# StefanHeng/Symbolic-Music-Generation

Measured on AMD Instinct MI355X. Metric: train tokens/sec (TransfoXL seq2048 bf16), whole job, higher is better.
Workload: dtype bf16; 1 GPU; TransfoXL 12L/768d H12 dh64 F3072 T=2048 M=2048 V=1190 cutoffs=[] (SURVEY C3, mode R: fresh zero mems); per_gpu_batch=64, global_batch=64, seq_len=2048, mem_len=2048, parallelism=dp1

## Files before the change

symbolic_music_generation_amd/csrc/gemm.hip:

```cpp
#include <stdlib.h>
#include <type_traits>
#include "common.h"
#include "musicxl_internal.h"

namespace {

constexpr int BM = 128, BK = 64;
constexpr int TILE_BYTES = BM * BK * 2;

struct GemmP {
    const bf16_t* A; const bf16_t* B; void* C;
    int M, N, K, lda, ldb, ldc;
    int ksplit;
    const float* bias;
    const bf16_t* aux;
    int ldaux;
    float alpha;
    int flags;
    unsigned long long seed; unsigned site; unsigned thresh; float drop_scale;
    int tiles_m, tiles_n;
    int bdiv;
    long long sA1, sA2, sB1, sB2, sC1, sC2;
    float* colsum;
    const bf16_t* hd_o; int hd_ldo, hd_T; float* hd_delta;
};
constexpr int GEMM_COLSUM_BIT = 0x80;
constexpr int GEMM_HEADDOT_BIT = 0x400;

typedef __attribute__((address_space(3))) bf16x4 lds_bf16x4;
typedef __attribute__((ext_vector_type(8))) __bf16 mfma_bf16x8;

__device__ __forceinline__ int swzT(int k) { return (k & 3) | (((k >> 3) & 1) << 2); }

template <bool T, int R_>
__device__ __forceinline__ void g2r(const bf16_t* __restrict__ X, int ld, int R, int kend, int r0, int k0, u32x4 (&v)[R_ / 32]) {
    const int t = threadIdx.x;
    constexpr int RC = R_ / 8;
#pragma unroll
    for (int i = 0; i < R_ / 32; i++) {
        const int c = t + i * 256;
        u32x4 z = {0u, 0u, 0u, 0u};
        if (!T) {
            const int row = c >> 3, kc = c & 7;
            const int gr = r0 + row, gk = k0 + kc * 8;
            const bool ok = (gr < R) && (gk < kend);
            v[i] = ok ? *reinterpret_cast<const u32x4*>(X + (size_t)gr * ld + gk) : z;
        } else {
            const int kr = c / RC, rc = c % RC;
            const int gk = k0 + kr, gr = r0 + rc * 8;
            const bool ok = (gk < kend) && (gr < R);
            v[i] = ok ? *reinterpret_cast<const u32x4*>(X + (size_t)gk * ld + gr) : z;
        }
    }
}

template <bool T, int R_>
__device__ __forceinline__ void r2s(char* base, const u32x4 (&v)[R_ / 32]) {
    const int t = threadIdx.x;
    constexpr int RC = R_ / 8;
#pragma unroll
    for (int i = 0; i < R_ / 32; i++) {
        const int c = t + i * 256;
        int off;
        if (!T) {
            const int row = c >> 3, kc = c & 7;
            off = row * 128 + ((kc ^ ((row >> 1) & 7)) << 4);
        } else {
            const int kr = c / RC, rc = c % RC;
            off = kr * (R_ * 2) + (((rc >> 1) ^ (swzT(kr) & (R_ / 16 - 1))) << 5) + ((rc & 1) << 4);
        }
        *reinterpret_cast<u32x4*>(base + off) = v[i];
    }
}

template <bool T, int R_>
__device__ __forceinline__ bf16x8 ldfrag(const char* base, int rb, int ks) {
    const int l = threadIdx.x & 63;
    const int g = l >> 4, li = l & 15;
    if (!T) {
        const int row = rb + li;
        const int chunk = ks * 4 + g;
        return *reinterpret_cast<const bf16x8*>(base + row * 128 + ((chunk ^ ((row >> 1) & 7)) << 4));
    } else {
        const int q = li >> 2, pp = li & 3;
        const int krow = ks * 32 + 8 * g + q;
        const int col = rb + 4 * pp;
        const int off = krow * (R_ * 2) + (((col >> 4) ^ (swzT(krow) & (R_ / 16 - 1))) << 5) + ((col & 15) << 1);
        const lds_bf16x4* p0 = (const lds_bf16x4*)(base + off);
        const lds_bf16x4* p1 = (const lds_bf16x4*)(base + off + 4 * (R_ * 2));
        bf16x4 lo = __builtin_amdgcn_ds_read_tr16_b64_v4i16((lds_bf16x4*)p0);
        bf16x4 hi = __builtin_amdgcn_ds_read_tr16_b64_v4i16((lds_bf16x4*)p1);
        bf16x8 r = {lo[0], lo[1], lo[2], lo[3], hi[0], hi[1], hi[2], hi[3]};
        return r;
    }
}

__device__ __forceinline__ void epilogue_vals(const GemmP& p, const int flags, const int m, const int n, const f32x4 a4_, float (&v)[4],
                                              const uint32_t* auxq = nullptr, const float* biasq = nullptr) {
#pragma unroll
            for (int r = 0; r < 4; r++) v[r] = a4_[r] * p.alpha;
            const bool full = (n + 3 < p.N);
            if ((flags & MXL_GEMM_BIAS) && biasq) {
#pragma unroll
                for (int r = 0; r < 4; r++) v[r] += biasq[r];
            } else if (flags & MXL_GEMM_BIAS) {
                if (full) {
                    const float b0 = p.bias[n], b1 = p.bias[n + 1], b2 = p.bias[n + 2], b3 = p.bias[n + 3];
                    v[0] += b0; v[1] += b1; v[2] += b2; v[3] += b3;
                } else {
#pragma unroll
                    for (int r = 0; r < 4; r++) if (n + r < p.N) v[r] += p.bias[n + r];
                }
            }
            if (flags & MXL_GEMM_RELU) {
#pragma unroll
                for (int r = 0; r < 4; r++) v[r] = fmaxf(v[r], 0.f);
            }
            if (flags & MXL_GEMM_DROPOUT) {
                const uint32_t i0 = (uint32_t)m * (uint32_t)p.N + (uint32_t)n;
                const uint32_t mix = mxl_hash32((uint32_t)p.seed ^ (p.site * 0x9E3779B9U)) + (uint32_t)(p.seed >> 32);
                const uint32_t h0 = i0 * 0x9E3779B1U;
                if (flags & MXL_GEMM_RELU) {
                    const uint32_t t16 = p.thresh >> 16;
#pragma unroll
                    for (int k = 0; k < 2; k++) {
                        const uint32_t h = mxl_hash32((h0 + (uint32_t)(2 * k) * 0x9E3779B1U) ^ mix);
                        v[2 * k] = ((h & 0xffffu) >= t16) ? v[2 * k] * p.drop_scale : 0.f;
                        v[2 * k + 1] = ((h >> 16) >= t16) ? v[2 * k + 1] * p.drop_scale : 0.f;
                    }
                } else
#pragma unroll
                for (int r = 0; r < 4; r++)
                    v[r] = (mxl_hash32((h0 + (uint32_t)r * 0x9E3779B1U) ^ mix) >= p.thresh) ? v[r] * p.drop_scale : 0.f;
            }
            if ((flags & MXL_GEMM_RELU_BWD) && auxq) {
                v[0] = bf2f((bf16_t)(auxq[0] & 0xffffu)) > 0.f ? v[0] : 0.f;
                v[1] = bf2f((bf16_t)(auxq[0] >> 16)) > 0.f ? v[1] : 0.f;
                v[2] = bf2f((bf16_t)(auxq[1] & 0xffffu)) > 0.f ? v[2] : 0.f;
                v[3] = bf2f((bf16_t)(auxq[1] >> 16)) > 0.f ? v[3] : 0.f;
            } else if (flags & MXL_GEMM_RELU_BWD) {
                if (full && ((p.ldaux & 3) == 0)) {
                    const bf16x4 a4 = *reinterpret_cast<const bf16x4*>(p.aux + (size_t)m * p.ldaux + n);
#pragma unroll
                    for (int r = 0; r < 4; r++) v[r] = bf2f((bf16_t)a4[r]) > 0.f ? v[r] : 0.f;
                } else {
#pragma unroll
                    for (int r = 0; r < 4; r++)
                        if (n + r < p.N) {
                            const float a = bf2f(p.aux[(size_t)m * p.ldaux + n + r]);
                            v[r] = a > 0.f ? v[r] : 0.f;
                        }
                }
            }
            if ((flags & MXL_GEMM_ADD_AUX) && auxq) {
                v[0] += bf2f((bf16_t)(auxq[0] & 0xffffu)); v[1] += bf2f((bf16_t)(auxq[0] >> 16));
                v[2] += bf2f((bf16_t)(auxq[1] & 0xffffu)); v[3] += bf2f((bf16_t)(auxq[1] >> 16));
            } else if (flags & MXL_GEMM_ADD_AUX) {
                if (full && ((p.ldaux & 3) == 0)) {
                    const bf16x4 a4 = *reinterpret_cast<const bf16x4*>(p.aux + (size_t)m * p.ldaux + n);
#pragma unroll
                    for (int r = 0; r < 4; r++) v[r] += bf2f((bf16_t)a4[r]);
                } else {
#pragma unroll
                    for (int r = 0; r < 4; r++)
                        if (n + r < p.N) v[r] += bf2f(p.aux[(size_t)m * p.ldaux + n + r]);
                }
            }
}
__device__ __forceinline__ void epilogue_store(const GemmP& p, const int flags, const int m, const int n, const float (&v)[4]) {
            const bool full = (n + 3 < p.N);
            if (flags & MXL_GEMM_OUT_F32_ATOMIC) {
                float* c = reinterpret_cast<float*>(p.C) + (size_t)m * p.ldc + n;
#pragma unroll
                for (int r = 0; r < 4; r++) if (n + r < p.N) atomicAdd(c + r, v[r]);
            } else if (flags & MXL_GEMM_OUT_F32) {
                float* c = reinterpret_cast<float*>(p.C) + (size_t)m * p.ldc + n;
                if (full && ((p.ldc & 3) == 0)) {
                    *reinterpret_cast<f32x4*>(c) = f32x4{v[0], v[1], v[2], v[3]};
                } else {
#pragma unroll
                    for (int r = 0; r < 4; r++) if (n + r < p.N) c[r] = v[r];
                }
            } else {
                bf16_t* c = reinterpret_cast<bf16_t*>(p.C) + (size_t)m * p.ldc + n;
                if (full && ((p.ldc & 3) == 0)) {
                    u32x2 o = {pack2bf(v[0], v[1]), pack2bf(v[2], v[3])};
                    if (flags & (1 << 30)) __builtin_nontemporal_store(o, reinterpret_cast<u32x2*>(c));
                    else *reinterpret_cast<u32x2*>(c) = o;
                } else {
#pragma unroll
                    for (int r = 0; r < 4; r++) if (n + r < p.N) c[r] = f2bf(v[r]);
                }
            }
}
__device__ __forceinline__ void epilogue_quad(const GemmP& p, const int flags, const int m, const int n, const f32x4 a4_) {
    float v[4];
    epilogue_vals(p, flags, m, n, a4_, v);
    epilogue_store(p, flags, m, n, v);
}
__device__ __forceinline__ u32x4 pair_aux_load(const GemmP& p, const int m, const int n, const int l) {
    const int acol = ((l >> 4) & 1) ? n + 16 - 4 : n;
    return *reinterpret_cast<const u32x4*>(p.aux + (size_t)m * p.ldaux + acol);
}
__device__ __forceinline__ void epilogue_pair_bf16(const GemmP& p, const int flags, const int m, const int n, const int l,
                                                   const f32x4 q0, const f32x4 q1, float* cs0 = nullptr, float* cs1 = nullptr,
                                                   const bool have_ax = false, const u32x4 axv = u32x4{0u, 0u, 0u, 0u},
                                                   const float* bq0 = nullptr, const float* bq1 = nullptr,
                                                   const int mask_mode = 0, uint32_t* mbits = nullptr, const int mshift = 0) {
    float v0[4], v1[4];
    if (mask_mode == 2) {
        const uint32_t b = *mbits >> mshift;
#pragma unroll
        for (int r = 0; r < 4; r++) {
            v0[r] = (b >> r) & 1u ? q0[r] * p.alpha : 0.f;
            v1[r] = (b >> (4 + r)) & 1u ? q1[r] * p.alpha : 0.f;
        }
    } else
    if ((flags & (MXL_GEMM_RELU_BWD | MXL_GEMM_ADD_AUX)) && (p.ldaux & 7) == 0 && (reinterpret_cast<uintptr_t>(p.aux) & 15) == 0) {
        const u32x4 ax = have_ax ? axv : pair_aux_load(p, m, n, l);
        const auto s0 = __builtin_amdgcn_permlane16_swap(ax[0], ax[2], false, false);
        const auto s1 = __builtin_amdgcn_permlane16_swap(ax[1], ax[3], false, false);
        const uint32_t aq0[2] = {s0[0], s1[0]}, aq1[2] = {s0[1], s1[1]};
        epilogue_vals(p, flags, m, n, q0, v0, aq0, bq0);
        epilogue_vals(p, flags, m, n + 16, q1, v1, aq1, bq1);
    } else {
        epilogue_vals(p, flags, m, n, q0, v0, nullptr, bq0);
        epilogue_vals(p, flags, m, n + 16, q1, v1, nullptr, bq1);
    }
    if (mask_mode == 1) {
        uint32_t b = 0;
#pragma unroll
        for (int r = 0; r < 4; r++) b |= (v0[r] > 0.f ? 1u << r : 0u) | (v1[r] > 0.f ? 16u << r : 0u);
        *mbits |= b << mshift;
    }
    if (cs0) {
#pragma unroll
        for (int r = 0; r < 4; r++) { cs0[r] += v0[r]; cs1[r] += v1[r]; }
    }
    unsigned a0 = pack2bf(v0[0], v0[1]), a1 = pack2bf(v0[2], v0[3]), b0 = pack2bf(v1[0], v1[1]), b1 = pack2bf(v1[2], v1[3]);
    const auto r0 = __builtin_amdgcn_permlane16_swap(a0, b0, false, false);
    const auto r1 = __builtin_amdgcn_permlane16_swap(a1, b1, false, false);
    const int col = ((l >> 4) & 1) ? n + 16 - 4 : n;
    bf16_t* c = reinterpret_cast<bf16_t*>(p.C) + (size_t)m * p.ldc + col;
    *reinterpret_cast<u32x4*>(c) = u32x4{r0[0], r1[0], r0[1], r1[1]};
}

__device__ __forceinline__ void epilogue_rowpair_bf16(const GemmP& p, const int flags, const int m, const int n, const int l,
                                                      const f32x4 q0, const f32x4 q1) {
    float v0[4], v1[4];
    epilogue_vals(p, flags, m, n, q0, v0);
    epilogue_vals(p, flags, m + 16, n, q1, v1);
    unsigned a0 = pack2bf(v0[0], v0[1]), a1 = pack2bf(v0[2], v0[3]), b0 = pack2bf(v1[0], v1[1]), b1 = pack2bf(v1[2], v1[3]);
    const auto r0 = __builtin_amdgcn_permlane16_swap(a0, b0, false, false);
    const auto r1 = __builtin_amdgcn_permlane16_swap(a1, b1, false, false);
    const bool odd = (l >> 4) & 1;
    bf16_t* c = reinterpret_cast<bf16_t*>(p.C) + (size_t)(odd ? m + 16 : m) * p.ldc + (odd ? n - 4 : n);
    *reinterpret_cast<u32x4*>(c) = u32x4{r0[0], r1[0], r0[1], r1[1]};
}

template <bool AT, bool BT, int BN_, bool SWAP = false>
__global__ __launch_bounds__(256, 2) void gemm_bf16_kernel(GemmP p) {
    constexpr int BN = BN_;
    constexpr int NF = BN / 32;
    constexpr int B_BYTES = BN * BK * 2;
    constexpr int STAGE = TILE_BYTES + B_BYTES;
    extern __shared__ __attribute__((aligned(16))) char smem[];
    const int nwg = p.tiles_m * p.tiles_n;
    int bid = blockIdx.x;
    {
        const int q = nwg >> 3, r = nwg & 7, xcd = bid & 7, idx = bid >> 3;
        bid = (xcd < r ? xcd * (q + 1) : r * (q + 1) + (xcd - r) * q) + idx;
    }
    if (gridDim.y > 1) {
        const long long b1 = blockIdx.y / p.bdiv, b2 = blockIdx.y % p.bdiv;
        p.A += b1 * p.sA1 + b2 * p.sA2;
        p.B += b1 * p.sB1 + b2 * p.sB2;
        const long long co = b1 * p.sC1 + b2 * p.sC2;
        if (p.flags & (MXL_GEMM_OUT_F32 | MXL_GEMM_OUT_F32_ATOMIC)) p.C = reinterpret_cast<float*>(p.C) + co;
        else p.C = reinterpret_cast<bf16_t*>(p.C) + co;
    }
    const int tm = bid / p.tiles_n, tn = bid % p.tiles_n;
    const int m0 = tm * BM, n0 = tn * BN;
    const int kbeg = blockIdx.z * p.ksplit;
    const int kend = min(p.K, kbeg + p.ksplit);
    const int nk = (kend - kbeg + BK - 1) / BK;

    const int wid = threadIdx.x >> 6, l = threadIdx.x & 63;
    const int wr = wid >> 1, wc = wid & 1;

    f32x4 acc[4][NF];
#pragma unroll
    for (int i = 0; i < 4; i++)
#pragma unroll
        for (int j = 0; j < NF; j++) acc[i][j] = f32x4{0.f, 0.f, 0.f, 0.f};

    u32x4 ra[4], rb[BN / 32];
    g2r<AT, 128>(p.A, p.lda, p.M, kend, m0, kbeg, ra);
    g2r<BT, BN>(p.B, p.ldb, p.N, kend, n0, kbeg, rb);
    r2s<AT, 128>(smem, ra);
    r2s<BT, BN>(smem + TILE_BYTES, rb);
    __syncthreads();

    int cur = 0;
    for (int kt = 0; kt < nk; kt++) {
        const bool more = (kt + 1 < nk);
        if (more) {
            g2r<AT, 128>(p.A, p.lda, p.M, kend, m0, kbeg + (kt + 1) * BK, ra);
            g2r<BT, BN>(p.B, p.ldb, p.N, kend, n0, kbeg + (kt + 1) * BK, rb);
        }
        const char* sa = smem + cur * STAGE;
        const char* sb = sa + TILE_BYTES;
#pragma unroll
        for (int ks = 0; ks < 2; ks++) {
            bf16x8 fa[4], fb[NF];
#pragma unroll
            for (int i = 0; i < 4; i++) fa[i] = ldfrag<AT, 128>(sa, wr * 64 + i * 16, ks);
#pragma unroll
            for (int j = 0; j < NF; j++) fb[j] = ldfrag<BT, BN>(sb, wc * (BN / 2) + j * 16, ks);
#pragma unroll
            for (int i = 0; i < 4; i++)
#pragma unroll
                for (int j = 0; j < NF; j++)
                    acc[i][j] = SWAP ? __builtin_amdgcn_mfma_f32_16x16x32_bf16(__builtin_bit_cast(mfma_bf16x8, fa[i]),
                                                                               __builtin_bit_cast(mfma_bf16x8, fb[j]), acc[i][j], 0, 0, 0)
                                     : __builtin_amdgcn_mfma_f32_16x16x32_bf16(__builtin_bit_cast(mfma_bf16x8, fb[j]),
                                                                               __builtin_bit_cast(mfma_bf16x8, fa[i]), acc[i][j], 0, 0, 0);
        }
        if (more) {
            char* da = smem + (cur ^ 1) * STAGE;
            r2s<AT, 128>(da, ra);
            r2s<BT, BN>(da + TILE_BYTES, rb);
        }
        __syncthreads();
        cur ^= 1;
    }

    if (SWAP) {
        float* C = reinterpret_cast<float*>(p.C);
#pragma unroll
        for (int i = 0; i < 4; i++)
#pragma unroll
            for (int j = 0; j < NF; j++) {
                const int n = n0 + wc * (BN / 2) + j * 16 + (l & 15);
#pragma unroll
                for (int r = 0; r < 4; r++) {
                    const int m = m0 + wr * 64 + i * 16 + (l >> 4) * 4 + r;
                    if (m < p.M && n < p.N) atomicAdd(C + (size_t)m * p.ldc + n, acc[i][j][r] * p.alpha);
                }
            }
        return;
    }
    const int flags = p.flags;
    const int mrow_l = l & 15, nq = (l >> 4) * 4;
#pragma unroll
    for (int i = 0; i < 4; i++) {
        const int m = m0 + wr * 64 + i * 16 + mrow_l;
        if (m >= p.M) continue;
#pragma unroll
        for (int j = 0; j < NF; j++) {
            const int n = n0 + wc * (BN / 2) + j * 16 + nq;
            if (n >= p.N) continue;
            epilogue_quad(p, flags, m, n, acc[i][j]);
        }
    }
}

constexpr int G2_OP_BYTES = 256 * 32 * 2;
constexpr int G2_STAGE = 2 * G2_OP_BYTES;
constexpr int G2_SMEM = 4 * G2_STAGE;

__device__ __forceinline__ int g2_swz(int rb) { return ((((rb ^ (rb >> 1)) & 1) << 1) | (rb >> 1)) & 3; }

typedef __attribute__((address_space(1))) const void* g2_gptr;
typedef __attribute__((address_space(3))) void* g2_lptr;

#ifndef NT_ABL
#define NT_ABL 0
#endif
template <int NFN, int EPI = -1>
__global__ __launch_bounds__(512) void gemm_nt256_kernel(GemmP p) {
    constexpr int BN = 64 * NFN;
    constexpr bool PF_ACROSS = !(EPI >= 0 && (EPI & (MXL_GEMM_DROPOUT | 0x100)));
    constexpr int WN = 4, WM = 2;
    constexpr int FM = 16 / WM, FN = BN / 16 / WN;
    extern __shared__ __attribute__((aligned(1024))) char smem[];
    const int nwg = p.tiles_m * p.tiles_n;
    const int G = gridDim.x;
    int bid = blockIdx.x;
    {
        const int q = G >> 3, r = G & 7, xcd = bid & 7, idx = bid >> 3;
        bid = (xcd < r ? xcd * (q + 1) : r * (q + 1) + (xcd - r) * q) + idx;
    }
    const int nk = p.K >> 5;
    const int my_tiles = (nwg - bid + G - 1) / G;
    const int S = my_tiles * nk;

    const int wid = __builtin_amdgcn_readfirstlane(threadIdx.x >> 6), l = threadIdx.x & 63;
    const int wr = wid / WN, wc = wid % WN;

    const __amdgpu_buffer_rsrc_t a_rsrc = __builtin_amdgcn_make_buffer_rsrc((void*)p.A, 0, -1, 0x00020000);
    const __amdgpu_buffer_rsrc_t b_rsrc = __builtin_amdgcn_make_buffer_rsrc((void*)p.B, 0, -1, 0x00020000);
    unsigned ga[2], gb[2];
    int gi = 0, i_t = 0, i_tile = bid;
    auto set_ptrs = [&](int tile) {
        const int tm = tile / p.tiles_n, tn = tile % p.tiles_n;
        const int kc = ((l & 3) ^ g2_swz(l >> 4)) * 8;
#pragma unroll
        for (int i = 0; i < 2; i++) {
            const int row = (8 * i + wid) * 16 + (l >> 2);
            ga[i] = (unsigned)min(tm * 256 + row, p.M - 1) * (unsigned)p.lda + kc;
            gb[i] = (unsigned)min(tn * BN + row, p.N - 1) * (unsigned)p.ldb + kc;
        }
    };
    set_ptrs(i_tile);
    auto issue_next = [&]() {
        char* st = smem + (gi & 3) * G2_STAGE;
        const int k0 = i_t << 5;
#pragma unroll
        for (int i = 0; i < 2; i++) {
            __builtin_amdgcn_raw_ptr_buffer_load_lds(a_rsrc, (g2_lptr)(st + (8 * i + wid) * 1024), 16, (int)((ga[i] + k0) * 2u), 0, 0, 0);
            if (NFN == 4 || i == 0 || wid < 4)
                __builtin_amdgcn_raw_ptr_buffer_load_lds(b_rsrc, (g2_lptr)(st + G2_OP_BYTES + (8 * i + wid) * 1024), 16,
                                                         (int)((gb[i] + k0) * 2u), 0, 0, 0);
        }
        gi++;
        if (++i_t == nk) {
            i_t = 0;
            i_tile += G;
            if (i_tile < nwg) set_ptrs(i_tile);
        }
    };
    const int fsw = ((l >> 4) ^ g2_swz((l >> 2) & 3)) << 4;
    const int a_off = (wr * (FM * 16) + (l & 15)) * 64 + fsw;
    const int b_off = G2_OP_BYTES + (wc * (FN * 16) + (l & 15)) * 64 + fsw;
    auto frags = [&](int g, bf16x8 (&fa)[FM], bf16x8 (&fb)[FN]) {
        const char* st = smem + (g & 3) * G2_STAGE;
#pragma unroll
        for (int j = 0; j < FN; j++) fb[j] = *reinterpret_cast<const bf16x8*>(st + b_off + j * 1024);
#pragma unroll
        for (int i = 0; i < FM; i++) fa[i] = *reinterpret_cast<const bf16x8*>(st + a_off + i * 1024);
    };

    f32x4 acc[FM][FN];
    issue_next();
    if (S > 1) issue_next();
    if (S > 2) issue_next();
    const bool three = (NFN == 3) && wid >= 4;
    if (S > 2) { if (three) asm volatile("s_waitcnt vmcnt(3)" ::: "memory"); else asm volatile("s_waitcnt vmcnt(4)" ::: "memory"); }
    else asm volatile("s_waitcnt vmcnt(0)" ::: "memory");
    __builtin_amdgcn_s_barrier();

    bf16x8 fa0[FM], fb0[FN], fa1[FM], fb1[FN];
    frags(0, fa0, fb0);
    __builtin_amdgcn_s_waitcnt(0xc07f);

    int g = 0;
    auto step = [&](bool first_of_later_tile, bool last_of_tile, bf16x8 (&fa)[FM], bf16x8 (&fb)[FN], bf16x8 (&na)[FM],
                    bf16x8 (&nb)[FN]) {
        const bool issued = gi < S;
        const bool late = wid >= 4;
        if (!late) {
            if (issued && !(NT_ABL & 1)) issue_next();
            if (g + 1 < S && !(last_of_tile && !PF_ACROSS) && !(NT_ABL & 2)) frags(g + 1, na, nb);
        }
        __builtin_amdgcn_s_setprio(1);
#pragma unroll
        for (int i = 0; i < FM; i++)
#pragma unroll
            for (int j = 0; j < FN; j++)
                acc[i][j] = __builtin_amdgcn_mfma_f32_16x16x32_bf16(__builtin_bit_cast(mfma_bf16x8, fb[j]),
                                                                    __builtin_bit_cast(mfma_bf16x8, fa[i]), acc[i][j], 0, 0, 0);
        __builtin_amdgcn_s_setprio(0);
        if (late) {
            __builtin_amdgcn_sched_barrier(0);
            if (g + 1 < S && !(last_of_tile && !PF_ACROSS) && !(NT_ABL & 2)) frags(g + 1, na, nb);
            if (issued && !(NT_ABL & 1)) issue_next();
        }
        if (last_of_tile || !issued) asm volatile("s_waitcnt vmcnt(0)" ::: "memory");
        else if (!first_of_later_tile) {
            if (three) asm volatile("s_waitcnt vmcnt(3)" ::: "memory"); else asm volatile("s_waitcnt vmcnt(4)" ::: "memory");
        }
        if (!(NT_ABL & 4)) __builtin_amdgcn_s_barrier();
        if (NT_ABL & 1) gi++;
        g++;
    };

    constexpr bool BIAS_INIT = EPI >= 0 && (EPI & MXL_GEMM_BIAS);
    const int flags = EPI >= 0 ? (BIAS_INIT ? EPI & ~MXL_GEMM_BIAS : EPI) : p.flags;
    if (EPI == 0 || BIAS_INIT) p.alpha = 1.f;
#pragma unroll 1
    for (int tile = bid; tile < nwg; tile += G) {
        if (BIAS_INIT) {
            const int nb0 = (tile % p.tiles_n) * BN + wc * (FN * 16) + (l >> 4) * 4;
#pragma unroll
            for (int j = 0; j < FN; j++) {
                f32x4 b4;
                const int n = nb0 + j * 16;
                if (n + 3 < p.N) b4 = *reinterpret_cast<const f32x4*>(p.bias + n);
                else
#pragma unroll
                    for (int r = 0; r < 4; r++) b4[r] = n + r < p.N ? p.bias[n + r] : 0.f;
#pragma unroll
                for (int i = 0; i < FM; i++) acc[i][j] = b4;
            }
        } else {
#pragma unroll
            for (int i = 0; i < FM; i++)
#pragma unroll
                for (int j = 0; j < FN; j++) acc[i][j] = f32x4{0.f, 0.f, 0.f, 0.f};
        }
#pragma unroll 1
        for (int t = 0; t < nk; t += 2) {
            step(t == 0 && tile != bid, false, fa0, fb0, fa1, fb1);
            step(false, t + 2 >= nk, fa1, fb1, fa0, fb0);
        }
        const int m0 = (tile / p.tiles_n) * 256, n0 = (tile % p.tiles_n) * BN;
        const bool pairs = !(flags & MXL_GEMM_OUT_F32) && n0 + BN <= p.N && m0 + 256 <= p.M && (p.ldc & 7) == 0 &&
                           (reinterpret_cast<uintptr_t>(p.C) & 15) == 0;
        if (pairs) {
            constexpr bool CS = EPI >= 0 && (EPI & GEMM_COLSUM_BIT) && !(FN & 1);
            float cs[CS ? FN : 1][4];
            if (CS) {
#pragma unroll
                for (int j = 0; j < FN; j++)
#pragma unroll
                    for (int r = 0; r < 4; r++) cs[j][r] = 0.f;
            }
            constexpr bool HA = false && EPI >= 0 && (EPI & (MXL_GEMM_RELU_BWD | MXL_GEMM_ADD_AUX)) && !(FN & 1);
            constexpr int MM = (EPI >= 0 && (EPI & 0x100)) ? 1 : (EPI >= 0 && (EPI & 0x200)) ? 2 : 0;
            uint32_t mb[4] = {0u, 0u, 0u, 0u};
            if (MM == 2) {
                const u32x4 t4 = *(reinterpret_cast<const u32x4*>(p.aux) + ((size_t)tile * 8 + wid) * 64 + l);
                mb[0] = t4[0]; mb[1] = t4[1]; mb[2] = t4[2]; mb[3] = t4[3];
            }
            const bool aux_ok = HA && (p.ldaux & 7) == 0 && (reinterpret_cast<uintptr_t>(p.aux) & 15) == 0;
            u32x4 axn[HA ? FN / 2 : 1];
#pragma unroll
            for (int i = 0; i < FM; i++) {
                const int m = m0 + wr * (FM * 16) + i * 16 + (l & 15);
                u32x4 axc[HA ? FN / 2 : 1];
                if (aux_ok) {
#pragma unroll
                    for (int j = 0; j + 1 < FN; j += 2) {
                        axc[j / 2] = i >= 2 ? axn[j / 2] : pair_aux_load(p, m, n0 + wc * (FN * 16) + j * 16 + (l >> 4) * 4, l);
                        if (i >= 1 && i + 1 < FM) axn[j / 2] = pair_aux_load(p, m + 16, n0 + wc * (FN * 16) + j * 16 + (l >> 4) * 4, l);
                    }
                }
#pragma unroll
                for (int j = 0; j + 1 < FN; j += 2)
                    epilogue_pair_bf16(p, flags & ~(GEMM_COLSUM_BIT | 0x300), m, n0 + wc * (FN * 16) + j * 16 + (l >> 4) * 4, l, acc[i][j], acc[i][j + 1],
                                       CS ? cs[CS ? j : 0] : nullptr, CS ? cs[CS ? j + 1 : 0] : nullptr,
                                       aux_ok, axc[HA ? j / 2 : 0], nullptr, nullptr,
                                       MM, &mb[(i * FN / 2 + j / 2) / 4], 8 * ((i * FN / 2 + j / 2) & 3));
                if ((FN & 1) && !(i & 1))
                    epilogue_rowpair_bf16(p, flags, m, n0 + wc * (FN * 16) + (FN - 1) * 16 + (l >> 4) * 4, l, acc[i][FN - 1],
                                          acc[(i + 1) % FM][FN - 1]);
                if (MM == 1) __builtin_amdgcn_sched_barrier(0);
            }
            if (MM == 1)
                *(reinterpret_cast<u32x4*>(const_cast<bf16_t*>(p.aux)) + ((size_t)tile * 8 + wid) * 64 + l) = u32x4{mb[0], mb[1], mb[2], mb[3]};
            if (CS) {
#pragma unroll
                for (int j = 0; j < FN; j++)
#pragma unroll
                    for (int r = 0; r < 4; r++) {
                        float v = cs[j][r];
                        v += __builtin_bit_cast(float, __builtin_amdgcn_update_dpp(0, __builtin_bit_cast(int, v), 0x128, 0xf, 0xf, false));
                        v += __builtin_bit_cast(float, __builtin_amdgcn_update_dpp(0, __builtin_bit_cast(int, v), 0x124, 0xf, 0xf, false));
                        v += __builtin_bit_cast(float, __builtin_amdgcn_update_dpp(0, __builtin_bit_cast(int, v), 0x122, 0xf, 0xf, false));
                        v += __builtin_bit_cast(float, __builtin_amdgcn_update_dpp(0, __builtin_bit_cast(int, v), 0x121, 0xf, 0xf, false));
                        cs[j][r] = v;
                    }
                if ((l & 15) == 0) {
#pragma unroll
                    for (int j = 0; j < FN; j++)
#pragma unroll
                        for (int r = 0; r < 4; r++) atomicAdd(p.colsum + n0 + wc * (FN * 16) + j * 16 + (l >> 4) * 4 + r, cs[j][r]);
                }
            }
        } else {
#pragma unroll
            for (int i = 0; i < FM; i++) {
                const int m = m0 + wr * (FM * 16) + i * 16 + (l & 15);
                if (m >= p.M) continue;
#pragma unroll
                for (int j = 0; j < FN; j++) {
                    const int n = n0 + wc * (FN * 16) + j * 16 + (l >> 4) * 4;
                    if (n >= p.N) continue;
                    epilogue_quad(p, flags, m, n, acc[i][j]);
                }
            }
        }
        if (!PF_ACROSS && g < S) {
            frags(g, fa0, fb0);
            __builtin_amdgcn_s_waitcnt(0xc07f);
        }
    }
}


#define W4S_(x) #x
#define W4S(x) W4S_(x)
#define W4_AREG(lo, hi) "{a[" W4S(lo) ":" W4S(hi) "]}"
#define W4_MFMA(i, j, lo, hi)                                                                                                     \
    do {                                                                                                                          \
        if (FIRST) asm volatile("v_mfma_f32_16x16x32_bf16 %0, %1, %2, 0" : "=" W4_AREG(lo, hi)(acc[i][j]) : "v"(fb[j]), "v"(fa[i])); \
        else asm volatile("v_mfma_f32_16x16x32_bf16 %0, %1, %2, %0" : "+" W4_AREG(lo, hi)(acc[i][j]) : "v"(fb[j]), "v"(fa[i]));     \
    } while (0)
#define W4_ACC_READ(i, j, r0, r1, r2, r3, lo, hi, q_)                                                                             \
    do {                                                                                                                          \
        float x0_, x1_, x2_, x3_;                                                                                                 \
        asm volatile("v_accvgpr_read_b32 %0, a" W4S(r0) "\n\tv_accvgpr_read_b32 %1, a" W4S(r1) "\n\tv_accvgpr_read_b32 %2, a" W4S(r2)  \
                     "\n\tv_accvgpr_read_b32 %3, a" W4S(r3)                                                                       \
                     : "=&v"(x0_), "=&v"(x1_), "=&v"(x2_), "=&v"(x3_) : W4_AREG(lo, hi)(acc[i][j]));                               \
        q_ = f32x4{x0_, x1_, x2_, x3_};                                                                                           \
    } while (0)
#include "gemm_w4_gen.inc"
template <int OFF>
__device__ __forceinline__ void w4_read(bf16x8& dst, uint32_t addr) {
    asm volatile("ds_read_b128 %0, %1 offset:%2" : "=v"(dst) : "v"(addr), "n"(OFF) : "memory");
}
template <int N>
__device__ __forceinline__ void w4_rd(bf16x8 (&na)[8], bf16x8 (&nb)[8], uint32_t aa, uint32_t bb) {
#if defined(W4_ABL) && (W4_ABL & 2)
    return;
#endif
    if (N < 8) w4_read<(N & 7) * 1024>(nb[N & 7], bb);
    else w4_read<(N & 7) * 1024>(na[N & 7], aa);
}
template <int EPI = -1>
__global__ __launch_bounds__(256, 1) void gemm_nt256w4_kernel(GemmP p) {
    constexpr int BN = 256, FM = 8, FN = 8;
    extern __shared__ __attribute__((aligned(1024))) char smem[];
    const int nwg = p.tiles_m * p.tiles_n;
    const int G = gridDim.x;
    int bid = blockIdx.x;
    {
        const int q = G >> 3, r = G & 7, xcd = bid & 7, idx = bid >> 3;
        bid = (xcd < r ? xcd * (q + 1) : r * (q + 1) + (xcd - r) * q) + idx;
    }
    const int nk = p.K >> 5;
    const int my_tiles = (nwg - bid + G - 1) / G;
    const int S = my_tiles * nk;
    const int wid = __builtin_amdgcn_readfirstlane(threadIdx.x >> 6), l = threadIdx.x & 63;
    const int wr = wid >> 1, wc = wid & 1;

    const __amdgpu_buffer_rsrc_t a_rsrc = __builtin_amdgcn_make_buffer_rsrc((void*)p.A, 0, -1, 0x00020000);
    const __amdgpu_buffer_rsrc_t b_rsrc = __builtin_amdgcn_make_buffer_rsrc((void*)p.B, 0, -1, 0x00020000);
    unsigned ga0, ga1, ga2, ga3, gb0, gb1, gb2, gb3;
    int gi = 0, i_t = 0, i_tile = bid;
    const int kc2 = ((l & 3) ^ g2_swz(l >> 4)) * 16;
#define W4_SET_PTRS(tile_)                                                                                                        \
    do {                                                                                                                          \
        const int tm_ = (tile_) / p.tiles_n, tn_ = (tile_) % p.tiles_n;                                                           \
        const int r0_ = wid * 16 + (l >> 2);                                                                                      \
        ga0 = (unsigned)min(tm_ * 256 + r0_, p.M - 1) * (unsigned)(p.lda * 2) + kc2;       \
        ga1 = (unsigned)min(tm_ * 256 + r0_ + 64, p.M - 1) * (unsigned)(p.lda * 2) + kc2;                                          \
        ga2 = (unsigned)min(tm_ * 256 + r0_ + 128, p.M - 1) * (unsigned)(p.lda * 2) + kc2;                                         \
        ga3 = (unsigned)min(tm_ * 256 + r0_ + 192, p.M - 1) * (unsigned)(p.lda * 2) + kc2;                                         \
        gb0 = (unsigned)min(tn_ * BN + r0_, p.N - 1) * (unsigned)(p.ldb * 2) + kc2;                                                \
// ... 318 lines not shown
}
static bool nt256_use192(int M, int N) {
    const int n_cu = gemm_n_cu();
    const int tm = (M + 255) / 256;
    const int t256 = tm * ((N + 255) / 256), t192 = tm * ((N + 191) / 192);
    const long long c256 = (long long)((t256 + n_cu - 1) / n_cu) * 256, c192 = (long long)((t192 + n_cu - 1) / n_cu) * 192;
    return c192 < c256;
}

extern "C" size_t mxl_gemm_relu_mask_bytes(int M, int N) {
    if (M <= 0 || N <= 0 || (M % 256) != 0 || (N % 256) != 0 || nt256_use192(M, N)) return 0;
    return (size_t)(M / 256) * (size_t)(N / 256) * 8 * 64 * 16;
}

static int gemm_launch(const void* A, const void* B, void* C, int M, int N, int K, int lda, int ldb, int ldc,
                       int transA, int transB, int flags, float alpha, const float* bias,
                       const void* aux, int ldaux, int ksplits,
                       float drop_p, unsigned long long seed, unsigned site, void* stream,
                       int batch, int bdiv, long long sA1, long long sA2, long long sB1, long long sB2,
                       long long sC1, long long sC2, float* colsum = nullptr, bool* colsum_fused = nullptr,
                       const void* hd_o = nullptr, int hd_ldo = 0, int hd_T = 0, float* hd_delta = nullptr, bool* hd_fused = nullptr) {
    MXL_CHECK_ARG(A && B && C && M > 0 && N > 0 && K > 0);
    g_last_nt_kernel = 0;
    MXL_CHECK_ARG((lda % 8) == 0 && (ldb % 8) == 0);
    MXL_CHECK_ARG(((uintptr_t)A % 16) == 0 && ((uintptr_t)B % 16) == 0);
    if (!transA || !transB) MXL_CHECK_ARG((K % 8) == 0);
    MXL_CHECK_ARG(transA ? lda >= ((M + 7) & ~7) : lda >= K);
    MXL_CHECK_ARG(transB ? ldb >= ((N + 7) & ~7) : ldb >= K);
    MXL_CHECK_ARG(ldc >= N);
    if (flags & MXL_GEMM_BIAS) MXL_CHECK_ARG(bias != nullptr);
    if (flags & (MXL_GEMM_SAVE_RELU_MASK | MXL_GEMM_RELU_BWD_BITS)) {
        MXL_CHECK_ARG(aux != nullptr && ((uintptr_t)aux & 15) == 0 && !(flags & (MXL_GEMM_RELU_BWD | MXL_GEMM_ADD_AUX)));
        MXL_CHECK_ARG(!((flags & MXL_GEMM_SAVE_RELU_MASK) && (flags & MXL_GEMM_RELU_BWD_BITS)));
        if (mxl_gemm_relu_mask_bytes(M, N) == 0 || transA || transB || batch != 1 || ksplits > 1 || (K % 64) != 0 || (ldc & 7) != 0 ||
            ((uintptr_t)C & 15) != 0 || (flags & (MXL_GEMM_OUT_F32 | MXL_GEMM_OUT_F32_ATOMIC)) || getenv("MXL_GEMM_NO256") ||
            (long long)M * lda >= (1ll << 31) || (long long)N * ldb >= (1ll << 31))
            return MXL_EUNSUPPORTED;
    }
    if (flags & (MXL_GEMM_RELU_BWD | MXL_GEMM_ADD_AUX)) MXL_CHECK_ARG(aux != nullptr && ldaux >= N);
    MXL_CHECK_ARG(!((flags & MXL_GEMM_RELU_BWD) && (flags & MXL_GEMM_ADD_AUX)));
    if (ksplits < 1) ksplits = 1;
    if (ksplits > 1) {
        MXL_CHECK_ARG(flags & MXL_GEMM_OUT_F32_ATOMIC);
        MXL_CHECK_ARG(!(flags & (MXL_GEMM_BIAS | MXL_GEMM_RELU | MXL_GEMM_DROPOUT | MXL_GEMM_RELU_BWD | MXL_GEMM_ADD_AUX)));
    }
    GemmP p;
    p.A = (const bf16_t*)A; p.B = (const bf16_t*)B; p.C = C;
    p.M = M; p.N = N; p.K = K; p.lda = lda; p.ldb = ldb; p.ldc = ldc;
    int ktiles = (K + BK - 1) / BK;
    int per = (ktiles + ksplits - 1) / ksplits;
    ksplits = (ktiles + per - 1) / per;
    p.ksplit = per * BK;
    p.bias = bias; p.aux = (const bf16_t*)aux; p.ldaux = ldaux; p.alpha = alpha; p.flags = flags;
    p.colsum = colsum;
    p.hd_o = (const bf16_t*)hd_o; p.hd_ldo = hd_ldo; p.hd_T = hd_T; p.hd_delta = hd_delta;
    p.seed = seed; p.site = site; p.thresh = dropout_thresh(drop_p);
    { static const bool nt = getenv("MXL_GEMM_NT") != nullptr; if (nt) p.flags |= (1 << 30); }
    p.drop_scale = drop_p > 0.f ? 1.f / (1.f - drop_p) : 1.f;
    if ((flags & MXL_GEMM_DROPOUT) && drop_p <= 0.f) p.flags &= ~MXL_GEMM_DROPOUT;
    if (p.flags & MXL_GEMM_DROPOUT) MXL_CHECK_ARG((unsigned long long)M * (unsigned long long)N <= 0xffffffffull);
    const int BN = (N <= 64) ? 64 : 128;
    p.tiles_m = (M + BM - 1) / BM; p.tiles_n = (N + BN - 1) / BN;
    MXL_CHECK_ARG(batch >= 1 && bdiv >= 1);
    if (batch > 1) {
        MXL_CHECK_ARG((sA1 % 8) == 0 && (sA2 % 8) == 0 && (sB1 % 8) == 0 && (sB2 % 8) == 0);
        MXL_CHECK_ARG(!(flags & (MXL_GEMM_RELU_BWD)));
    }
    p.bdiv = bdiv; p.sA1 = sA1; p.sA2 = sA2; p.sB1 = sB1; p.sB2 = sB2; p.sC1 = sC1; p.sC2 = sC2;
    hipStream_t s = (hipStream_t)stream;
    if (!transA && !transB && batch == 1 && ksplits == 1 && (K % 64) == 0 && M >= 256 && N >= 192 &&
        (long long)M * lda < (1ll << 31) && (long long)N * ldb < (1ll << 31) &&
        !(flags & MXL_GEMM_OUT_F32_ATOMIC) && !getenv("MXL_GEMM_NO256")) {
        const int n_cu = gemm_n_cu();
        const int tm = (M + 255) / 256;
        const bool use192 = nt256_use192(M, N);
        p.tiles_m = tm; p.tiles_n = use192 ? (N + 191) / 192 : (N + 255) / 256;
        const int ntile = p.tiles_m * p.tiles_n;
        dim3 grid(ntile < n_cu ? ntile : n_cu);
#define MXL_NT256_LAUNCH(EPI_)                                                                                                   \
    do {                                                                                                                         \
        static bool attr_e = false;                                                                                              \
        if (!attr_e) {                                                                                                           \
            hipError_t e = hipFuncSetAttribute(reinterpret_cast<const void*>(&gemm_nt256_kernel<4, EPI_>),                         \
                                               hipFuncAttributeMaxDynamicSharedMemorySize, G2_SMEM);                             \
            if (e != hipSuccess) return (int)e;                                                                                  \
            e = hipFuncSetAttribute(reinterpret_cast<const void*>(&gemm_nt256_kernel<3, EPI_>),                                    \
                                    hipFuncAttributeMaxDynamicSharedMemorySize, G2_SMEM);                                        \
            if (e != hipSuccess) return (int)e;                                                                                  \
            attr_e = true;                                                                                                       \
        }                                                                                                                        \
        if (use192) hipLaunchKernelGGL((gemm_nt256_kernel<3, EPI_>), grid, dim3(512), G2_SMEM, s, p);                       \
        else hipLaunchKernelGGL((gemm_nt256_kernel<4, EPI_>), grid, dim3(512), G2_SMEM, s, p);                                     \
        g_last_nt_kernel = use192 ? 2 : 1;                                                                                      \
    } while (0)
        const char* w4_env = getenv("MXL_GEMM_W4");
        const bool w4 = !(w4_env && w4_env[0] == '0');
#define MXL_NT256W4_LAUNCH(EPI_)                                                                                                 \
    do {                                                                                                                         \
        static bool attr_w = false;                                                                                              \
        if (!attr_w) {                                                                                                           \
            hipError_t e = hipFuncSetAttribute(reinterpret_cast<const void*>(&gemm_nt256w4_kernel<EPI_>),                          \
                                               hipFuncAttributeMaxDynamicSharedMemorySize, G2_SMEM);                             \
            if (e != hipSuccess) return (int)e;                                                                                  \
            attr_w = true;                                                                                                       \
        }                                                                                                                        \
        hipLaunchKernelGGL((gemm_nt256w4_kernel<EPI_>), grid, dim3(256), G2_SMEM, s, p);                                          \
        g_last_nt_kernel = 3;                                                                                                    \
    } while (0)
        const bool w4_ok = w4 && !use192 && (M % 256) == 0 && (N % 256) == 0 && (ldc & 7) == 0 && ((uintptr_t)C & 15) == 0 && p.alpha == 1.f;
        if (w4_ok && p.flags == 0 && hd_delta && (N % 128) == 0 && hd_T > 0 && (M % hd_T) == 0 && (hd_ldo & 7) == 0 && ((uintptr_t)hd_o & 15) == 0) {
            MXL_NT256W4_LAUNCH(GEMM_HEADDOT_BIT);
            *hd_fused = true;
        }
        else if (w4_ok && p.flags == 0) MXL_NT256W4_LAUNCH(0);
        else if (w4_ok && p.flags == MXL_GEMM_BIAS) MXL_NT256W4_LAUNCH(MXL_GEMM_BIAS);
        else if (p.flags == 0 && p.alpha == 1.f) MXL_NT256_LAUNCH(0);
        else if (p.alpha != 1.f && (p.flags & MXL_GEMM_BIAS) && !(p.flags & (MXL_GEMM_SAVE_RELU_MASK | MXL_GEMM_RELU_BWD_BITS))) MXL_NT256_LAUNCH(-1);
        else if (p.alpha != 1.f && (p.flags & MXL_GEMM_SAVE_RELU_MASK)) return MXL_EUNSUPPORTED;
        else if (p.flags == MXL_GEMM_BIAS) MXL_NT256_LAUNCH(MXL_GEMM_BIAS);
        else if (p.flags == (MXL_GEMM_BIAS | MXL_GEMM_OUT_F32)) MXL_NT256_LAUNCH(MXL_GEMM_BIAS | MXL_GEMM_OUT_F32);
        else if (p.flags == (MXL_GEMM_BIAS | MXL_GEMM_RELU)) MXL_NT256_LAUNCH(MXL_GEMM_BIAS | MXL_GEMM_RELU);
        else if (p.flags == (MXL_GEMM_BIAS | MXL_GEMM_RELU | MXL_GEMM_DROPOUT)) MXL_NT256_LAUNCH(MXL_GEMM_BIAS | MXL_GEMM_RELU | MXL_GEMM_DROPOUT);
        else if (p.flags == (MXL_GEMM_BIAS | MXL_GEMM_RELU | MXL_GEMM_DROPOUT | MXL_GEMM_SAVE_RELU_MASK))
            MXL_NT256_LAUNCH(MXL_GEMM_BIAS | MXL_GEMM_RELU | MXL_GEMM_DROPOUT | MXL_GEMM_SAVE_RELU_MASK);
        else if (p.flags == (MXL_GEMM_BIAS | MXL_GEMM_RELU | MXL_GEMM_SAVE_RELU_MASK))
            MXL_NT256_LAUNCH(MXL_GEMM_BIAS | MXL_GEMM_RELU | MXL_GEMM_SAVE_RELU_MASK);
        else if (p.flags == MXL_GEMM_RELU_BWD_BITS && colsum) {
            MXL_NT256_LAUNCH(MXL_GEMM_RELU_BWD_BITS | GEMM_COLSUM_BIT);
            *colsum_fused = true;
        }
        else if (p.flags == MXL_GEMM_RELU_BWD_BITS) MXL_NT256_LAUNCH(MXL_GEMM_RELU_BWD_BITS);
        else if (p.flags & (MXL_GEMM_SAVE_RELU_MASK | MXL_GEMM_RELU_BWD_BITS)) return MXL_EUNSUPPORTED;
        else if (p.flags == MXL_GEMM_RELU_BWD && colsum && !use192 && (M % 256) == 0 && (N % 256) == 0 && (ldc & 7) == 0 &&
                 ((uintptr_t)C & 15) == 0) {
            MXL_NT256_LAUNCH(MXL_GEMM_RELU_BWD | GEMM_COLSUM_BIT);
            *colsum_fused = true;
        }
        else if (p.flags == MXL_GEMM_RELU_BWD) MXL_NT256_LAUNCH(MXL_GEMM_RELU_BWD);
        else if (p.flags == MXL_GEMM_ADD_AUX) MXL_NT256_LAUNCH(MXL_GEMM_ADD_AUX);
        else if (p.flags == (MXL_GEMM_ADD_AUX | MXL_GEMM_DROPOUT)) MXL_NT256_LAUNCH(MXL_GEMM_ADD_AUX | MXL_GEMM_DROPOUT);
        else if (p.flags == (MXL_GEMM_BIAS | MXL_GEMM_ADD_AUX)) MXL_NT256_LAUNCH(MXL_GEMM_BIAS | MXL_GEMM_ADD_AUX);
        else if (p.flags == (MXL_GEMM_BIAS | MXL_GEMM_ADD_AUX | MXL_GEMM_DROPOUT))
            MXL_NT256_LAUNCH(MXL_GEMM_BIAS | MXL_GEMM_ADD_AUX | MXL_GEMM_DROPOUT);
        else MXL_NT256_LAUNCH(-1);
#undef MXL_NT256_LAUNCH
#undef MXL_NT256W4_LAUNCH
        MXL_LAUNCH_CHECK();
        return MXL_OK;
    }
    if (transA && transB && batch == 1 && p.flags == MXL_GEMM_OUT_F32_ATOMIC && (M % 256) == 0 && (N % 256) == 0 && (K % 32) == 0 &&
        K >= 8192 && (long long)K * lda < (1ll << 31) && (long long)K * ldb < (1ll << 31) && ((uintptr_t)C % 16) == 0 &&
        !getenv("MXL_GEMM_NO_TT256")) {
        static bool attr_tt = false;
        if (!attr_tt) {
            hipError_t e = hipFuncSetAttribute(reinterpret_cast<const void*>(&gemm_tt256_kernel),
                                               hipFuncAttributeMaxDynamicSharedMemorySize, G2_SMEM);
            if (e != hipSuccess) return (int)e;
            attr_tt = true;
        }
        const int n_cu_tt = gemm_n_cu();
        p.tiles_m = M / 256; p.tiles_n = N / 256;
        const int ntile = p.tiles_m * p.tiles_n;
        int ks = n_cu_tt / ntile;
        if (ks < 1) ks = 1;
        const int steps = K / 32;
        if (ks > steps / 64) ks = steps / 64 > 0 ? steps / 64 : 1;
        const int per_steps = (steps + ks - 1) / ks;
        ks = (steps + per_steps - 1) / per_steps;
        p.ksplit = per_steps * 32;
        hipLaunchKernelGGL(gemm_tt256_kernel, dim3(ntile * ks), dim3(512), G2_SMEM, s, p);
        MXL_LAUNCH_CHECK();
        return MXL_OK;
    }
    dim3 grid(p.tiles_m * p.tiles_n, batch, ksplits), block(256);
#define MXL_GEMM_LAUNCH(AT_, BT_)                                                                                          \
// ... 55 lines not shown
```

Measured before the change: 863,200 tokens/s.

## Accumulate GEMM column sums in LDS with column-grouped tile order

In the persistent NT256 GEMM with the column-sum epilogue, workgroups now visit tiles so that consecutive tiles share the same column block. Per-tile column partials are reduced with a transposing DPP butterfly into an LDS buffer. Global atomics are issued only when the column block changes, instead of per wave per tile, which cuts atomic traffic to the colsum vector. This costs extra LDS, barriers and a more involved tile schedule. It also adds compile-time ablation switches (NT_EPI_ABL, default off) and replaces the lane id with an mbcnt-based one.

```diff
diff --git a/symbolic_music_generation_amd/csrc/gemm.hip b/symbolic_music_generation_amd/csrc/gemm.hip
--- a/symbolic_music_generation_amd/csrc/gemm.hip
+++ b/symbolic_music_generation_amd/csrc/gemm.hip
@@ -29,6 +29,10 @@
 
 typedef __attribute__((address_space(3))) bf16x4 lds_bf16x4;
 typedef __attribute__((ext_vector_type(8))) __bf16 mfma_bf16x8;
+
+#ifndef NT_EPI_ABL
+#define NT_EPI_ABL 0
+#endif
 
 __device__ __forceinline__ int swzT(int k) { return (k & 3) | (((k >> 3) & 1) << 2); }
 
@@ -124,7 +128,8 @@
                     const uint32_t t16 = p.thresh >> 16;
 #pragma unroll
                     for (int k = 0; k < 2; k++) {
-                        const uint32_t h = mxl_hash32((h0 + (uint32_t)(2 * k) * 0x9E3779B1U) ^ mix);
+                        const uint32_t hx = (h0 + (uint32_t)(2 * k) * 0x9E3779B1U) ^ mix;
+                        const uint32_t h = (NT_EPI_ABL & 1) ? hx : mxl_hash32(hx);
                         v[2 * k] = ((h & 0xffffu) >= t16) ? v[2 * k] * p.drop_scale : 0.f;
                         v[2 * k + 1] = ((h >> 16) >= t16) ? v[2 * k + 1] * p.drop_scale : 0.f;
                     }
@@ -212,8 +217,8 @@
         const uint32_t b = *mbits >> mshift;
 #pragma unroll
         for (int r = 0; r < 4; r++) {
-            v0[r] = (b >> r) & 1u ? q0[r] * p.alpha : 0.f;
-            v1[r] = (b >> (4 + r)) & 1u ? q1[r] * p.alpha : 0.f;
+            v0[r] = ((NT_EPI_ABL & 8) || ((b >> r) & 1u)) ? q0[r] * p.alpha : 0.f;
+            v1[r] = ((NT_EPI_ABL & 8) || ((b >> (4 + r)) & 1u)) ? q1[r] * p.alpha : 0.f;
         }
     } else
     if ((flags & (MXL_GEMM_RELU_BWD | MXL_GEMM_ADD_AUX)) && (p.ldaux & 7) == 0 && (reinterpret_cast<uintptr_t>(p.aux) & 15) == 0) {
@@ -227,7 +232,7 @@
         epilogue_vals(p, flags, m, n, q0, v0, nullptr, bq0);
         epilogue_vals(p, flags, m, n + 16, q1, v1, nullptr, bq1);
     }
-    if (mask_mode == 1) {
+    if (mask_mode == 1 && !(NT_EPI_ABL & 2)) {
         uint32_t b = 0;
 #pragma unroll
         for (int r = 0; r < 4; r++) b |= (v0[r] > 0.f ? 1u << r : 0u) | (v1[r] > 0.f ? 16u << r : 0u);
@@ -368,8 +373,15 @@
 constexpr int G2_OP_BYTES = 256 * 32 * 2;
 constexpr int G2_STAGE = 2 * G2_OP_BYTES;
 constexpr int G2_SMEM = 4 * G2_STAGE;
+constexpr int G2_CS_BYTES = 2 * 256 * 4;
+constexpr int g2_smem_bytes(int epi) { return epi >= 0 && (epi & GEMM_COLSUM_BIT) ? G2_SMEM + G2_CS_BYTES : G2_SMEM; }
 
 __device__ __forceinline__ int g2_swz(int rb) { return ((((rb ^ (rb >> 1)) & 1) << 1) | (rb >> 1)) & 3; }
+__device__ __forceinline__ int g2_lane_here() {
+    int x;
+    asm volatile("v_mbcnt_lo_u32_b32 %0, -1, 0\n\tv_mbcnt_hi_u32_b32 %0, -1, %0" : "=v"(x));
+    return x;
+}
 
 typedef __attribute__((address_space(1))) const void* g2_gptr;
 typedef __attribute__((address_space(3))) void* g2_lptr;
@@ -394,6 +406,20 @@
     const int nk = p.K >> 5;
     const int my_tiles = (nwg - bid + G - 1) / G;
     const int S = my_tiles * nk;
+    constexpr bool CS = EPI >= 0 && (EPI & GEMM_COLSUM_BIT) && !(NFN & 1);
+    const int cs_whole = CS ? (G / p.tiles_n) * p.tiles_n : 0;
+    const int cs_col = CS ? bid % p.tiles_n : 0;
+    auto tile_of = [&](int k) -> int {
+        const int base = k * G;
+        if (CS && bid < cs_whole && base + G <= nwg) {
+            int r = cs_col - base % p.tiles_n;
+            if (r < 0) r += p.tiles_n;
+            return base + (bid - cs_col) + r;
+        }
+        return base + bid;
+    };
+    float* const cs_lds = reinterpret_cast<float*>(smem + G2_SMEM);
+    if (CS) cs_lds[threadIdx.x] = 0.f;
 
     const int wid = __builtin_amdgcn_readfirstlane(threadIdx.x >> 6), l = threadIdx.x & 63;
     const int wr = wid / WN, wc = wid % WN;
@@ -401,7 +427,7 @@
     const __amdgpu_buffer_rsrc_t a_rsrc = __builtin_amdgcn_make_buffer_rsrc((void*)p.A, 0, -1, 0x00020000);
     const __amdgpu_buffer_rsrc_t b_rsrc = __builtin_amdgcn_make_buffer_rsrc((void*)p.B, 0, -1, 0x00020000);
     unsigned ga[2], gb[2];
-    int gi = 0, i_t = 0, i_tile = bid;
+    int gi = 0, i_t = 0, i_tile = bid, i_round = 0;
     auto set_ptrs = [&](int tile) {
         const int tm = tile / p.tiles_n, tn = tile % p.tiles_n;
         const int kc = ((l & 3) ^ g2_swz(l >> 4)) * 8;
@@ -426,8 +452,12 @@
         gi++;
         if (++i_t == nk) {
             i_t = 0;
-            i_tile += G;
-            if (i_tile < nwg) set_ptrs(i_tile);
+            if (CS) {
+                if (++i_round < my_tiles) set_ptrs(tile_of(i_round));
+            } else {
+                i_tile += G;
+                if (i_tile < nwg) set_ptrs(i_tile);
+            }
         }
     };
     const int fsw = ((l >> 4) ^ g2_swz((l >> 2) & 3)) << 4;
@@ -448,6 +478,7 @@
     const bool three = (NFN == 3) && wid >= 4;
     if (S > 2) { if (three) asm volatile("s_waitcnt vmcnt(3)" ::: "memory"); else asm volatile("s_waitcnt vmcnt(4)" ::: "memory"); }
     else asm volatile("s_waitcnt vmcnt(0)" ::: "memory");
+    if (CS) asm volatile("s_waitcnt lgkmcnt(0)" ::: "memory");
     __builtin_amdgcn_s_barrier();
 
     bf16x8 fa0[FM], fb0[FN], fa1[FM], fb1[FN];
@@ -488,8 +519,10 @@
     constexpr bool BIAS_INIT = EPI >= 0 && (EPI & MXL_GEMM_BIAS);
     const int flags = EPI >= 0 ? (BIAS_INIT ? EPI & ~MXL_GEMM_BIAS : EPI) : p.flags;
     if (EPI == 0 || BIAS_INIT) p.alpha = 1.f;
+    int rd = 0;
 #pragma unroll 1
-    for (int tile = bid; tile < nwg; tile += G) {
+    for (int tile0 = bid; tile0 < nwg; tile0 += G, rd++) {
+        const int tile = CS ? tile_of(rd) : tile0;
         if (BIAS_INIT) {
             const int nb0 = (tile % p.tiles_n) * BN + wc * (FN * 16) + (l >> 4) * 4;
 #pragma unroll
@@ -511,14 +544,13 @@
         }
 #pragma unroll 1
         for (int t = 0; t < nk; t += 2) {
-            step(t == 0 && tile != bid, false, fa0, fb0, fa1, fb1);
+            step(t == 0 && tile0 != bid, false, fa0, fb0, fa1, fb1);
             step(false, t + 2 >= nk, fa1, fb1, fa0, fb0);
         }
         const int m0 = (tile / p.tiles_n) * 256, n0 = (tile % p.tiles_n) * BN;
         const bool pairs = !(flags & MXL_GEMM_OUT_F32) && n0 + BN <= p.N && m0 + 256 <= p.M && (p.ldc & 7) == 0 &&
                            (reinterpret_cast<uintptr_t>(p.C) & 15) == 0;
         if (pairs) {
-            constexpr bool CS = EPI >= 0 && (EPI & GEMM_COLSUM_BIT) && !(FN & 1);
             float cs[CS ? FN : 1][4];
             if (CS) {
 #pragma unroll
@@ -530,7 +562,7 @@
             constexpr int MM = (EPI >= 0 && (EPI & 0x100)) ? 1 : (EPI >= 0 && (EPI & 0x200)) ? 2 : 0;
             uint32_t mb[4] = {0u, 0u, 0u, 0u};
             if (MM == 2) {
-                const u32x4 t4 = *(reinterpret_cast<const u32x4*>(p.aux) + ((size_t)tile * 8 + wid) * 64 + l);
+                const u32x4 t4 = *(reinterpret_cast<const u32x4*>(p.aux) + ((size_t)tile * 8 + wid) * 64 + g2_lane_here());
                 mb[0] = t4[0]; mb[1] = t4[1]; mb[2] = t4[2]; mb[3] = t4[3];
             }
             const bool aux_ok = HA && (p.ldaux & 7) == 0 && (reinterpret_cast<uintptr_t>(p.aux) & 15) == 0;
@@ -558,24 +590,36 @@
                 if (MM == 1) __builtin_amdgcn_sched_barrier(0);
             }
             if (MM == 1)
-                *(reinterpret_cast<u32x4*>(const_cast<bf16_t*>(p.aux)) + ((size_t)tile * 8 + wid) * 64 + l) = u32x4{mb[0], mb[1], mb[2], mb[3]};
+                *(reinterpret_cast<u32x4*>(const_cast<bf16_t*>(p.aux)) + ((size_t)tile * 8 + wid) * 64 + g2_lane_here()) = u32x4{mb[0], mb[1], mb[2], mb[3]};
             if (CS) {
-#pragma unroll
-                for (int j = 0; j < FN; j++)
-#pragma unroll
-                    for (int r = 0; r < 4; r++) {
-                        float v = cs[j][r];
-                        v += __builtin_bit_cast(float, __builtin_amdgcn_update_dpp(0, __builtin_bit_cast(int, v), 0x128, 0xf, 0xf, false));
-                        v += __builtin_bit_cast(float, __builtin_amdgcn_update_dpp(0, __builtin_bit_cast(int, v), 0x124, 0xf, 0xf, false));
-                        v += __builtin_bit_cast(float, __builtin_amdgcn_update_dpp(0, __builtin_bit_cast(int, v), 0x122, 0xf, 0xf, false));
-                        v += __builtin_bit_cast(float, __builtin_amdgcn_update_dpp(0, __builtin_bit_cast(int, v), 0x121, 0xf, 0xf, false));
-                        cs[j][r] = v;
+                const int ll = g2_lane_here();
+                float t8[8], t4[4], t2[2];
+#define G2_DPP_ADD(mine, other, ctrl) ((mine) + __builtin_bit_cast(float, __builtin_amdgcn_update_dpp(0, __builtin_bit_cast(int, (other)), ctrl, 0xf, 0xf, false)))
+#pragma unroll
+                for (int k = 0; k < 8; k++) {
+                    const float a = cs[k >> 2][k & 3], b = cs[2 + (k >> 2)][k & 3];
+                    t8[k] = G2_DPP_ADD((ll & 8) ? b : a, (ll & 8) ? a : b, 0x140);
+                }
+#pragma unroll
+                for (int k = 0; k < 4; k++) t4[k] = G2_DPP_ADD((ll & 4) ? t8[4 + k] : t8[k], (ll & 4) ? t8[k] : t8[4 + k], 0x141);
+#pragma unroll
+                for (int k = 0; k < 2; k++) t2[k] = G2_DPP_ADD((ll & 2) ? t4[2 + k] : t4[k], (ll & 2) ? t4[k] : t4[2 + k], 0x1b);
+                const float mine = G2_DPP_ADD((ll & 1) ? t2[1] : t2[0], (ll & 1) ? t2[0] : t2[1], 0xb1);
+#undef G2_DPP_ADD
+                float* const w = cs_lds + wr * 256 + wc * (FN * 16) + ((ll & 15) >> 2) * 16 + (ll >> 4) * 4 + (ll & 3);
+                *w += mine;
+                const int next_tn = rd + 1 < my_tiles ? tile_of(rd + 1) % p.tiles_n : -1;
+                if (next_tn != tile % p.tiles_n) {
+                    asm volatile("s_waitcnt lgkmcnt(0)" ::: "memory");
+                    __builtin_amdgcn_s_barrier();
+                    const int tx = wid * 64 + g2_lane_here();
+                    if (tx < 256) {
+                        const float v = cs_lds[tx] + cs_lds[256 + tx];
+                        cs_lds[tx] = 0.f;
+                        cs_lds[256 + tx] = 0.f;
+                        if (!(NT_EPI_ABL & 16)) atomicAdd(p.colsum + n0 + tx, v);
                     }
-                if ((l & 15) == 0) {
-#pragma unroll
-                    for (int j = 0; j < FN; j++)
-#pragma unroll
-                        for (int r = 0; r < 4; r++) atomicAdd(p.colsum + n0 + wc * (FN * 16) + j * 16 + (l >> 4) * 4 + r, cs[j][r]);
+                    asm volatile("s_waitcnt lgkmcnt(0)" ::: "memory");
                 }
             }
         } else {
@@ -1060,15 +1104,16 @@
         static bool attr_e = false;                                                                                              \
         if (!attr_e) {                                                                                                           \
             hipError_t e = hipFuncSetAttribute(reinterpret_cast<const void*>(&gemm_nt256_kernel<4, EPI_>),                         \
-                                               hipFuncAttributeMaxDynamicSharedMemorySize, G2_SMEM);                             \
+                                               hipFuncAttributeMaxDynamicSharedMemorySize, g2_smem_bytes(EPI_));                 \
             if (e != hipSuccess) return (int)e;                                                                                  \
             e = hipFuncSetAttribute(reinterpret_cast<const void*>(&gemm_nt256_kernel<3, EPI_>),                                    \
-                                    hipFuncAttributeMaxDynamicSharedMemorySize, G2_SMEM);                                        \
+                                    hipFuncAttributeMaxDynamicSharedMemorySize, g2_smem_bytes(EPI_));                            \
             if (e != hipSuccess) return (int)e;                                                                                  \
             attr_e = true;                                                                                                       \
         }                                                                                                                        \
-        if (use192) hipLaunchKernelGGL((gemm_nt256_kernel<3, EPI_>), grid, dim3(512), G2_SMEM, s, p);                       \
-        else hipLaunchKernelGGL((gemm_nt256_kernel<4, EPI_>), grid, dim3(512), G2_SMEM, s, p);                                     \
+        const int smem_e = g2_smem_bytes(EPI_);                                                                                  \
+        if (use192) hipLaunchKernelGGL((gemm_nt256_kernel<3, EPI_>), grid, dim3(512), smem_e, s, p);                        \
+        else hipLaunchKernelGGL((gemm_nt256_kernel<4, EPI_>), grid, dim3(512), smem_e, s, p);                                      \
         g_last_nt_kernel = use192 ? 2 : 1;                                                                                      \
     } while (0)
         const char* w4_env = getenv("MXL_GEMM_W4");
```

Result: slower. 850,200 tokens/s (-1.5%).
